# AIS-Bonn/stillleben

Measured on AMD Instinct MI355X. Metric: scenes/sec (settle + 640x480 6-ch GT render), 20-obj YCB-like, higher is better.
Workload: dtype f32; 1 GPU; C2: 20 of 21 procedural YCB-like objects (8k verts/16k tris, 1024^2 texture each) per scene; per step and GPU 32768 scenes are staged (random stack), settled (100 frames x 4 substeps), framed (camera, light, shadow matrix) and rendered at 640x480 (rgb, coord+depth, class, instance, normals; shadows on, SSAO on) -- all four stages inside the timed region; render_chunk=512, objects=20, settle_streams=1, render_streams=2, pair_contact_budget=0, parallelism=1 GPU

## Files before the change

### stillleben_amd/csrc/slhip_raster_walk.h

```cpp
#pragma once

#include <stdint.h>

#if defined(__HIPCC__)
#define SLHIP_RW_HD __host__ __device__ __forceinline__
#else
#define SLHIP_RW_HD inline
#endif

namespace slhip_raster {

constexpr long long kNarrowMax = 1ll << 29;

SLHIP_RW_HD bool narrow_ok(long long ex, long long ey)
{
    const long long m = ex > ey ? ex : ey;
    return 256 * m <= kNarrowMax && ex * ey <= kNarrowMax;
}

template <class I>
SLHIP_RW_HD I edge_value(const int* X, const int* Y, int flipped, int i, int cx, int cy)
{
    const int a = (i + 1) % 3, b = (i + 2) % 3;
    const I e = I(X[b] - X[a]) * I(cy - Y[a]) - I(Y[b] - Y[a]) * I(cx - X[a]);
    return flipped ? -e : e;
}

template <class I>
struct Walk {
    I e[3];
    I row[3];
    I sx[3];
    I sy[3];
    int bias[3];

    SLHIP_RW_HD void start(const int* X, const int* Y, int flipped, const int* bias_, int px, int py)
    {
        const int cx = 256 * px + 128, cy = 256 * py + 128;
#pragma unroll
        for (int i = 0; i < 3; ++i) {
            const int a = (i + 1) % 3, b = (i + 2) % 3;
            const I dx = I(-256) * I(Y[b] - Y[a]), dy = I(256) * I(X[b] - X[a]);
            sx[i] = flipped ? -dx : dx;
            sy[i] = flipped ? -dy : dy;
            bias[i] = bias_[i];
            row[i] = edge_value<I>(X, Y, flipped, i, cx, cy) + I(bias_[i]);
            e[i] = row[i];
        }
    }
    SLHIP_RW_HD void step_x()
    {
        e[0] += sx[0]; e[1] += sx[1]; e[2] += sx[2];
    }
    SLHIP_RW_HD void next_row()
    {
        row[0] += sy[0]; row[1] += sy[1]; row[2] += sy[2];
        e[0] = row[0]; e[1] = row[1]; e[2] = row[2];
    }
    SLHIP_RW_HD bool inside() const { return (e[0] | e[1] | e[2]) >= I(0); }
    SLHIP_RW_HD I numerator(int i) const { return e[i] - I(bias[i]); }
};

template <class I>
SLHIP_RW_HD bool cover(const int* X, const int* Y, int flipped, const int* bias, int px, int py, I* num)
{
    const int cx = 256 * px + 128, cy = 256 * py + 128;
    bool in = true;
#pragma unroll
    for (int i = 0; i < 3; ++i) {
        const I e = edge_value<I>(X, Y, flipped, i, cx, cy);
        in = in && (e + I(bias[i]) >= I(0));
        num[i] = e;
    }
    return in;
}

}
```

### stillleben_amd/csrc/slhip_render.hip

```cpp
#include <algorithm>
#include <cmath>
#include <cstring>
#include <vector>
#include <type_traits>
#include "slhip_common.h"
#include "slhip_cubemap.h"
#include "slhip_raster_walk.h"
#include "slhip_tile_queue.h"

#ifndef SLHIP_RENDER_WAVES
#define SLHIP_RENDER_WAVES 0
#endif
#ifndef SLHIP_SHADE_WAVES
#define SLHIP_SHADE_WAVES 0
#endif
#ifndef SLHIP_SSAO_WAVES
#define SLHIP_SSAO_WAVES 0
#endif
#if SLHIP_RENDER_WAVES > 0
#define SLHIP_LIGHT_KERNEL __attribute__((amdgpu_waves_per_eu(1, SLHIP_RENDER_WAVES)))
#else
#define SLHIP_LIGHT_KERNEL
#endif
#if SLHIP_RENDER_WAVES > 0
// ... 396 lines not shown

__device__ __forceinline__ int wrapi(int i, int n)
{
    if ((n & (n - 1)) == 0) return i & (n - 1);
    int m = i % n;
    return m < 0 ? m + n : m;
}

__device__ __forceinline__ int wrap_coord(int i, int n, unsigned mode)
{
    if (mode == 1u) return min(max(i, 0), n - 1);
    if (mode == 2u) {
        const int m = wrapi(i, 2 * n);
        return m < n ? m : 2 * n - 1 - m;
    }
    return wrapi(i, n);
}

__device__ __forceinline__ void texel_rgba(const uint8_t* __restrict__ pool_tex, unsigned lvl, int w, int x, int y, float* out)
{
    const uchar4 t = *reinterpret_cast<const uchar4*>(pool_tex + (lvl + 4u * ((unsigned)y * (unsigned)w + (unsigned)x)));
    out[0] = slhip::unorm8(t.x); out[1] = slhip::unorm8(t.y); out[2] = slhip::unorm8(t.z); out[3] = slhip::unorm8(t.w);
}

__device__ __forceinline__ void tex_level(const uint8_t* __restrict__ pool_tex, unsigned lvl, int w, int h, unsigned sampler,
                                          bool linear, float u, float v, float* out)
{
    const unsigned ws = SLHIP_SAMPLER_WRAP_S(sampler), wt = SLHIP_SAMPLER_WRAP_T(sampler);
    if (!linear) {
        texel_rgba(pool_tex, lvl, w, wrap_coord((int)floorf(u * (float)w), w, ws), wrap_coord((int)floorf(v * (float)h), h, wt), out);
        return;
    }
    const float x = fmaf(u, (float)w, -0.5f), y = fmaf(v, (float)h, -0.5f);
    const float fx = floorf(x), fy = floorf(y);
    const float ax = x - fx, ay = y - fy;
    const int x0 = wrap_coord((int)fx, w, ws), y0 = wrap_coord((int)fy, h, wt);
    const int x1 = wrap_coord((int)fx + 1, w, ws), y1 = wrap_coord((int)fy + 1, h, wt);
    float c00[4], c10[4], c01[4], c11[4];
    texel_rgba(pool_tex, lvl, w, x0, y0, c00); texel_rgba(pool_tex, lvl, w, x1, y0, c10);
    texel_rgba(pool_tex, lvl, w, x0, y1, c01); texel_rgba(pool_tex, lvl, w, x1, y1, c11);
#pragma unroll
    for (int c = 0; c < 4; ++c) {
        const float top = fmaf(ax, c10[c] - c00[c], c00[c]), bot = fmaf(ax, c11[c] - c01[c], c01[c]);
        out[c] = fmaf(ay, bot - top, top);
    }
}

__device__ __forceinline__ unsigned tex_level_off(unsigned tex, int w0, int h0, int l, int& w, int& h)
{
    unsigned off = tex;
    w = w0; h = h0;
    for (int k = 0; k < l; ++k) {
        off += 4u * (unsigned)w * (unsigned)h;
        w = max(1, w >> 1); h = max(1, h >> 1);
    }
    return off;
}

__device__ __forceinline__ float det_log2(float x)
{
    const unsigned bits = __float_as_uint(x);
    const int e = (int)(bits >> 23) - 127;
    const float t = __uint_as_float((bits & 0x7fffffu) | 0x3f800000u) - 1.0f;
    float q = 0.02049034833908081f;
    q = fmaf(q, t, -0.09606625884771347f);
    q = fmaf(q, t, 0.2155885398387909f);
    q = fmaf(q, t, -0.33924779295921326f);
    q = fmaf(q, t, 0.4777059257030487f);
    q = fmaf(q, t, -0.721162736415863f);
    q = fmaf(q, t, 1.4426932334899902f);
    return fmaf(q, t, (float)e);
}

__device__ __forceinline__ void tex_sample(const uint8_t* __restrict__ pool_tex, unsigned tex, int w, int h, unsigned sampler, float u,
                                           float v, float dudx, float dvdx, float dudy, float dvdy, float* out)
{
    const unsigned mip = SLHIP_SAMPLER_MIP(sampler);
    const float ax = dudx * (float)w, bx = dvdx * (float)h, ay = dudy * (float)w, by = dvdy * (float)h;
    const float rx = sqrtf(fmaf(bx, bx, ax * ax)), ry = sqrtf(fmaf(by, by, ay * ay));
    const float rho = fmaxf(rx, ry);
    const bool magnify = !(rho > 1.0f);
    if (magnify || mip == 0u) {
        tex_level(pool_tex, tex, w, h, sampler, (sampler & (magnify ? SLHIP_SAMPLER_MAG_LINEAR : SLHIP_SAMPLER_MIN_LINEAR)) != 0u, u, v, out);
        return;
    }
    const int top = 31 - __clz(max(max(w, h), 1));
    const float lambda = fminf(det_log2(rho), (float)top);
    const bool lin = (sampler & SLHIP_SAMPLER_MIN_LINEAR) != 0u;
    int lw, lh;
    if (mip == 1u) {
        const int l = min((int)ceilf(lambda + 0.5f) - 1, top);
        const unsigned p = tex_level_off(tex, w, h, max(l, 0), lw, lh);
        tex_level(pool_tex, p, lw, lh, sampler, lin, u, v, out);
        return;
    }
    const int l0 = min((int)floorf(lambda), top), l1 = min(l0 + 1, top);
    const float f = lambda - (float)l0;
    float a[4], b[4];
    const unsigned p0 = tex_level_off(tex, w, h, l0, lw, lh);
    tex_level(pool_tex, p0, lw, lh, sampler, lin, u, v, a);
    if (l1 == l0 || f == 0.0f) {
#pragma unroll
        for (int c = 0; c < 4; ++c) out[c] = a[c];
        return;
    }
    const unsigned p1 = p0 + 4u * (unsigned)lw * (unsigned)lh;
    lw = max(1, lw >> 1); lh = max(1, lh >> 1);
    tex_level(pool_tex, p1, lw, lh, sampler, lin, u, v, b);
#pragma unroll
    for (int c = 0; c < 4; ++c) out[c] = fmaf(f, b[c] - a[c], a[c]);
}

__device__ __forceinline__ void bary_at(const Setup& t, const float* b0, const float* b1, const float* b2, int px, int py, float* b)
{
    const int cx = 256 * px + 128, cy = 256 * py + 128;
    float l[3];
    const float fa = (float)t.area2;
#pragma unroll
    for (int i = 0; i < 3; ++i) {
        const int a = (i + 1) % 3, c = (i + 2) % 3;
        long long e = (long long)(t.X[c] - t.X[a]) * (long long)(cy - t.Y[a]) - (long long)(t.Y[c] - t.Y[a]) * (long long)(cx - t.X[a]);
        if (t.flipped) e = -e;
        l[i] = (float)e / fa;
    }
    const float pw0 = l[0] * t.invw[0], pw1 = l[1] * t.invw[1], pw2 = l[2] * t.invw[2];
    const float sw = (pw0 + pw1) + pw2;
    const float bs[3] = {pw0 * (1.0f / sw), pw1 * (1.0f / sw), pw2 * (1.0f / sw)};
#pragma unroll
    for (int k = 0; k < 3; ++k) b[k] = fmaf(bs[2], b2[k], fmaf(bs[1], b1[k], bs[0] * b0[k]));
}

__device__ __forceinline__ void tex_rect_bilinear(const uint8_t* __restrict__ tex, int w, int h, float xt, float yt, float* out)
{
    const float x = xt - 0.5f, y = yt - 0.5f;
    const float fx = floorf(x), fy = floorf(y);
    const float ax = x - fx, ay = y - fy;
    const int x0 = min(max((int)fx, 0), w - 1), x1 = min(max((int)fx + 1, 0), w - 1);
    const int y0 = (h - 1) - min(max((int)fy, 0), h - 1), y1 = (h - 1) - min(max((int)fy + 1, 0), h - 1);
    const uchar4 t00 = reinterpret_cast<const uchar4*>(tex)[(size_t)y0 * w + x0];
    const uchar4 t10 = reinterpret_cast<const uchar4*>(tex)[(size_t)y0 * w + x1];
    const uchar4 t01 = reinterpret_cast<const uchar4*>(tex)[(size_t)y1 * w + x0];
    const uchar4 t11 = reinterpret_cast<const uchar4*>(tex)[(size_t)y1 * w + x1];
    const unsigned char c00[4] = {t00.x, t00.y, t00.z, t00.w}, c10[4] = {t10.x, t10.y, t10.z, t10.w};
    const unsigned char c01[4] = {t01.x, t01.y, t01.z, t01.w}, c11[4] = {t11.x, t11.y, t11.z, t11.w};
#pragma unroll
    for (int c = 0; c < 4; ++c) {
        const float a = slhip::unorm8(c00[c]), b = slhip::unorm8(c10[c]);
        const float cc = slhip::unorm8(c01[c]), d = slhip::unorm8(c11[c]);
        const float top = fmaf(ax, b - a, a), bot = fmaf(ax, d - cc, cc);
        out[c] = fmaf(ay, bot - top, top);
    }
}

struct MainTarget {
    unsigned long long* vis;
    const float* peel;
    int W;
    unsigned prim;
    bool need_attr;
    const float* camz;
    const float* bary;
    const float* uv;
    const uint8_t* pool_tex;
    unsigned tex;
    int tex_w, tex_h;
    unsigned tex_sampler;
    float base_alpha, alpha_cutoff;

    __device__ __forceinline__ void emit(const Setup& t, int px, int py, const float* l) const
    {
        const float z = interp(l, t.z[0], t.z[1], t.z[2]);
        if (!(z >= 0.0f && z <= 1.0f)) return;
        const unsigned d24 = depth24(z);
        if (d24 >= 0xFFFFFFu) return;
        const unsigned long long key = ((unsigned long long)d24 << 32) | prim;
        unsigned long long* slot = vis + (size_t)py * W + px;
        if (need_attr && __builtin_nontemporal_load(slot) <= key) return;
        if (need_attr) {
            const float pw0 = l[0] * t.invw[0], pw1 = l[1] * t.invw[1], pw2 = l[2] * t.invw[2];
            const float sw = (pw0 + pw1) + pw2;
            const float bs[3] = {pw0 * (1.0f / sw), pw1 * (1.0f / sw), pw2 * (1.0f / sw)};
            float b[3];
#pragma unroll
            for (int k = 0; k < 3; ++k)
                b[k] = fmaf(bs[2], bary[6 + k], fmaf(bs[1], bary[3 + k], bs[0] * bary[k]));
            if (peel) {
                const float cz = interp(b, camz[0], camz[1], camz[2]);
                if (cz - 0.00001f <= peel[4 * ((size_t)py * W + px) + 3]) return;
            }
            if (pool_tex) {
                const float u = interp(b, uv[0], uv[2], uv[4]);
                const float v = interp(b, uv[1], uv[3], uv[5]);
                float bx[3], by[3];
                bary_at(t, bary, bary + 3, bary + 6, px + 1, py, bx);
                bary_at(t, bary, bary + 3, bary + 6, px, py + 1, by);
                float tc[4];
                tex_sample(pool_tex, tex, tex_w, tex_h, tex_sampler, u, v, interp(bx, uv[0], uv[2], uv[4]) - u, interp(bx, uv[1], uv[3], uv[5]) - v,
                           interp(by, uv[0], uv[2], uv[4]) - u, interp(by, uv[1], uv[3], uv[5]) - v, tc);
                if (base_alpha * tc[3] < alpha_cutoff) return;
            }
        }
        atomicMin(slot, key);
    }
};

#ifndef SLHIP_SHADOW_WINDOW
#define SLHIP_SHADOW_WINDOW 64
#endif
#ifndef SLHIP_SHADOW_WINDOW_PITCH
#define SLHIP_SHADOW_WINDOW_PITCH SLHIP_SHADOW_WINDOW
#endif
struct ShadowTarget {
    unsigned* sm;
    int W;
    unsigned* win;
    int wx0, wy0;
    unsigned wnx, wny;
    __device__ __forceinline__ void emit(const Setup& t, int px, int py, const float* l) const
    {
        const float z = interp(l, t.z[0], t.z[1], t.z[2]);
        if (!(z >= 0.0f && z <= 1.0f)) return;
        const unsigned bits = __float_as_uint(z);
#if SLHIP_SHADOW_WINDOW
        const unsigned ux = (unsigned)(px - wx0), uy = (unsigned)(py - wy0);
        if (ux < wnx && uy < wny) {
            atomicMin(win + uy * SLHIP_SHADOW_WINDOW_PITCH + ux, bits);
            return;
        }
#endif
        unsigned* slot = sm + (size_t)py * W + px;
        atomicMin(slot, bits);
    }
};

struct QueueShare {
    const slhip_tq::Entry* entries;
    slhip_tq::Walk walk;
    __device__ __forceinline__ QueueShare(const unsigned* __restrict__ queue, unsigned capacity)
    {
        const unsigned wave = (unsigned)__builtin_amdgcn_readfirstlane((int)((blockIdx.x * blockDim.x + threadIdx.x) >> 6));
        const unsigned n_waves = (gridDim.x * blockDim.x) >> 6;
        entries = reinterpret_cast<const slhip_tq::Entry*>(queue + slhip_tq::kHeaderWords);
        walk.first(slhip_tq::plan_of(queue[0], queue[1], queue[2], capacity), entries, n_waves, wave);
    }
};

struct TilePixels {
    unsigned ntx, tx, ty;
    int px0, py0;
    __device__ __forceinline__ TilePixels(const slhip_tq::Entry& en, unsigned k0, unsigned lane)
    {
        ntx = slhip_tq::ntx(en);
        ty = k0 / ntx; tx = k0 - ty * ntx;
        px0 = (int)((en.t0 & 0xFFFFu) << 3) + (int)(lane & 7);
        py0 = (int)((en.t0 >> 16) << 3) + (int)(lane >> 3);
    }
    __device__ __forceinline__ void next(int& px, int& py)
    {
        px = px0 + (int)(tx << 3); py = py0 + (int)(ty << 3);
        if (++tx == ntx) { tx = 0u; ++ty; }
    }
};

template <class I, class Target>
__device__ __forceinline__ void raster_bbox_as(const Setup& t, const Target& tgt)
{
    slhip_raster::Walk<I> w;
    w.start(t.X, t.Y, t.flipped, t.bias, t.xmin, t.ymin);
    const float fa = (float)(I)t.area2;
    const int bw = t.xmax - t.xmin + 1, n = bw * (t.ymax - t.ymin + 1);
    int px = t.xmin, py = t.ymin;
    for (int k = 0; k < n; ++k) {
        if (w.inside()) {
            float l[3];
            l[0] = (float)w.numerator(0) / fa;
            l[1] = (float)w.numerator(1) / fa;
            l[2] = (float)w.numerator(2) / fa;
            tgt.emit(t, px, py, l);
        }
        if (px == t.xmax) {
            px = t.xmin; ++py;
            w.next_row();
        } else {
            ++px;
            w.step_x();
        }
    }
}

template <class Target>
__device__ __forceinline__ void raster_bbox(const Setup& t, const Target& tgt, int wide)
{
    if (!wide && __all(t.narrow)) {
        raster_bbox_as<int>(t, tgt);
    } else {
        const int bw = t.xmax - t.xmin + 1, n = bw * (t.ymax - t.ymin + 1);
        int px = t.xmin, py = t.ymin;
        for (int k = 0; k < n; ++k) {
            float l[3];
            if (coverage_as<long long>(t, px, py, l)) tgt.emit(t, px, py, l);
            if (px == t.xmax) { px = t.xmin; ++py; } else ++px;
        }
    }
}

template <class Target>
__device__ __forceinline__ void raster_or_enqueue(const Setup& t, const Target& tgt, unsigned* queue,
                                                  unsigned capacity, unsigned draw, unsigned tri_sub,
                                                  unsigned scene_aux, int small_area, int wide = 0)
{
    const int bw = t.xmax - t.xmin + 1, bh = t.ymax - t.ymin + 1;
    bool in_place = bw * bh <= small_area;
    if (!in_place) {
        const unsigned tx0 = (unsigned)(t.xmin >> 3), ty0 = (unsigned)(t.ymin >> 3);
        const unsigned ntx = (unsigned)(t.xmax >> 3) - tx0 + 1u, nty = (unsigned)(t.ymax >> 3) - ty0 + 1u;
        const unsigned n = ntx * nty;
        const slhip_tq::Slot s =
            slhip_tq::slot_of(atomicAdd(reinterpret_cast<unsigned long long*>(queue), slhip_tq::reservation(n)), n, capacity);
        if (s.carried) atomicOr(queue + 2, 1u);
        if (s.fits) {
            uint4* e = reinterpret_cast<uint4*>(queue + slhip_tq::kHeaderWords) + slhip_tq::kUnitsPerEntry * (size_t)s.index;
            e[0] = make_uint4(draw, tri_sub, scene_aux, s.tile_base);
            e[1] = make_uint4(tx0 | (ty0 << 16), s.carried ? 0u : (ntx | (nty << 16)), 0u, 0u);
        }
        in_place = !s.fits || s.carried;
    }
    if (in_place) raster_bbox(t, tgt, wide);
}

template <bool kAttr>
__device__ __forceinline__ void raster_chunk(unsigned chunk, const slhip_mesh_pool& pool, const slhip_scene* __restrict__ scenes,
                                             const slhip_draw* __restrict__ draws,
                                             const slhip_chunk* __restrict__ chunks, int W, int H,
                                             const float* __restrict__ depth_peel,
                                             unsigned long long* __restrict__ vis, unsigned* queue,
                                             unsigned capacity, const float4* __restrict__ clipbuf,
                                             const uint4* __restrict__ screen, int small_area, int wide)
{
    const slhip_chunk ch = chunks[chunk];
    if (threadIdx.x >= ch.count) return;
    const slhip_scene* sc = scenes + ch.scene;
    const slhip_draw* dr = draws + ch.draw;
    const bool alpha_test = (dr->flags & SLHIP_DRAW_ALPHA_TEST) && (dr->flags & SLHIP_DRAW_HAS_BASE_TEX);
    if ((alpha_test || depth_peel != nullptr) != kAttr) return;
    const unsigned tri = ch.first_tri + threadIdx.x;
    const unsigned* ip = pool.d_idx + dr->idx_base + 3 * (size_t)tri;
    const unsigned vi[3] = {ip[0], ip[1], ip[2]};
    const size_t P = (size_t)W * H;
    MainTarget tgt;
    tgt.vis = vis + (size_t)ch.scene * P;
    tgt.W = W;
    tgt.prim = dr->prim_base + tri;
    tgt.need_attr = kAttr;
    tgt.peel = nullptr;
    tgt.pool_tex = nullptr;

    if constexpr (!kAttr) {
        tgt.camz = nullptr; tgt.uv = nullptr; tgt.bary = nullptr;
        const uint4 s0 = screen[dr->clip_base + vi[0]], s1 = screen[dr->clip_base + vi[1]], s2 = screen[dr->clip_base + vi[2]];
        if (screen_all_inside(s0, s1, s2)) {
            Setup t;
            if (setup_from_screen(s0, s1, s2, W, H, t)) raster_or_enqueue(t, tgt, queue, capacity, ch.draw, tri, ch.scene, small_area, wide);
            return;
        }
        ClipVert cv[3];
#pragma unroll
        for (int k = 0; k < 3; ++k) {
            const float4 c4 = clipbuf[dr->clip_base + vi[k]];
            cv[k].clip[0] = c4.x; cv[k].clip[1] = c4.y; cv[k].clip[2] = c4.z; cv[k].clip[3] = c4.w;
            cv[k].bary[0] = cv[k].bary[1] = cv[k].bary[2] = 0.0f;
        }
        ClipVert poly[4];
        const int n = clip_near(cv, poly);
#pragma unroll
        for (int sub = 0; sub < 2; ++sub) {
            if (sub >= n - 2) break;
            Setup t;
            if (!setup_tri(poly[0].clip, poly[sub + 1].clip, poly[sub + 2].clip, W, H, t)) continue;
            raster_or_enqueue(t, tgt, queue, capacity, ch.draw, tri | ((unsigned)sub << 31), ch.scene, small_area, wide);
        }
    } else {
        ClipVert cv[3];
        float camz[3] = {0.0f, 0.0f, 0.0f};
#pragma unroll
        for (int k = 0; k < 3; ++k) {
            const float4 c4 = clipbuf[dr->clip_base + vi[k]];
            cv[k].clip[0] = c4.x; cv[k].clip[1] = c4.y; cv[k].clip[2] = c4.z; cv[k].clip[3] = c4.w;
            if (depth_peel) {
                float unused[4];
                vertex_clip(pool, sc, dr, dr->vtx_base + vi[k], unused, camz[k]);
            }
            cv[k].bary[0] = k == 0 ? 1.0f : 0.0f;
            cv[k].bary[1] = k == 1 ? 1.0f : 0.0f;
            cv[k].bary[2] = k == 2 ? 1.0f : 0.0f;
        }
        ClipVert poly[4];
        const int n = clip_near(cv, poly);
        if (n == 0) return;
        tgt.peel = depth_peel ? depth_peel + 4 * (size_t)ch.scene * P : nullptr;
        float uvs[6] = {0, 0, 0, 0, 0, 0};
        if (alpha_test) {
#pragma unroll
            for (int k = 0; k < 3; ++k) {
                const float2 uv = reinterpret_cast<const float2*>(pool.d_uv)[dr->vtx_base + vi[k]];
                uvs[2 * k] = uv.x; uvs[2 * k + 1] = uv.y;
            }
            tgt.pool_tex = pool.d_tex; tgt.tex = dr->tex_offset;
            tgt.tex_w = (int)dr->tex_w; tgt.tex_h = (int)dr->tex_h;
            tgt.tex_sampler = dr->tex_sampler[0];
        }
        tgt.camz = camz;
        tgt.uv = uvs;
        tgt.base_alpha = dr->base_color[3];
        tgt.alpha_cutoff = dr->alpha_cutoff;
#pragma unroll
        for (int sub = 0; sub < 2; ++sub) {
            if (sub >= n - 2) break;
            Setup t;
            if (!setup_tri(poly[0].clip, poly[sub + 1].clip, poly[sub + 2].clip, W, H, t)) continue;
            float bary[9];
#pragma unroll
            for (int k = 0; k < 3; ++k) {
                bary[k] = poly[0].bary[k];
                bary[3 + k] = poly[sub + 1].bary[k];
                bary[6 + k] = poly[sub + 2].bary[k];
            }
            tgt.bary = bary;
            for (int py = t.ymin; py <= t.ymax; ++py)
                for (int px = t.xmin; px <= t.xmax; ++px) {
                    float l[3];
                    if (coverage(t, px, py, l)) tgt.emit(t, px, py, l);
                }
        }
    }
}

template <bool kAttr>
__global__ __launch_bounds__(256) SLHIP_LIGHT_KERNEL void k_raster(slhip_mesh_pool pool, const slhip_scene* __restrict__ scenes,
                                                const slhip_draw* __restrict__ draws,
                                                const slhip_chunk* __restrict__ chunks, unsigned n_chunks, int W, int H,
                                                const float* __restrict__ depth_peel,
                                                unsigned long long* __restrict__ vis, unsigned* queue,
                                                unsigned capacity, const float4* __restrict__ clipbuf,
                                                const uint4* __restrict__ screen, int small_area, int wide)
{
    for (unsigned c = blockIdx.x; c < n_chunks; c += gridDim.x)
        raster_chunk<kAttr>(c, pool, scenes, draws, chunks, W, H, depth_peel, vis, queue, capacity, clipbuf, screen, small_area, wide);
}

__global__ __launch_bounds__(256) SLHIP_LIGHT_KERNEL void k_large(slhip_mesh_pool pool, const slhip_scene* __restrict__ scenes,
                                               const slhip_draw* __restrict__ draws, int W, int H,
                                               unsigned long long* __restrict__ vis,
                                               const unsigned* __restrict__ queue, unsigned capacity,
                                               const float4* __restrict__ clipbuf, const uint4* __restrict__ screen)
{
    const QueueShare q(queue, capacity);
    const unsigned lane = threadIdx.x & 63;
    for (unsigned e = q.walk.e0; e < q.walk.e1; ++e) {
        const slhip_tq::Entry en = q.entries[e];
        if (q.walk.done(en)) break;
        unsigned k0, k1;
        if (!q.walk.tiles(en, k0, k1)) continue;
        Setup t;
        const slhip_draw* dr = draws + en.draw;
        const unsigned tri = en.tri_sub & 0x7FFFFFFFu;
        const int sub = (int)(en.tri_sub >> 31);
        const unsigned* ip = pool.d_idx + dr->idx_base + 3 * (size_t)tri;
        ClipVert cv[3];
        const uint4 s0 = screen[dr->clip_base + ip[0]], s1 = screen[dr->clip_base + ip[1]], s2 = screen[dr->clip_base + ip[2]];
        const bool cached = screen_all_inside(s0, s1, s2);
        if (cached && (sub != 0 || !setup_from_screen(s0, s1, s2, W, H, t))) continue;
        if (!cached) {
#pragma unroll
            for (int k = 0; k < 3; ++k) {
                const float4 c4 = clipbuf[dr->clip_base + ip[k]];
                cv[k].clip[0] = c4.x; cv[k].clip[1] = c4.y; cv[k].clip[2] = c4.z; cv[k].clip[3] = c4.w;
                cv[k].bary[0] = cv[k].bary[1] = cv[k].bary[2] = 0.0f;
            }
            ClipVert poly[4];
            const int n = clip_near(cv, poly);
            if (sub > n - 3) continue;
            const ClipVert& pb = sub == 0 ? poly[1] : poly[2];
            const ClipVert& pc = sub == 0 ? poly[2] : poly[3];
            if (!setup_tri(poly[0].clip, pb.clip, pc.clip, W, H, t)) continue;
        }
        MainTarget tgt;
        tgt.vis = vis + (size_t)en.scene_aux * W * H;
        tgt.peel = nullptr;
        tgt.W = W;
        tgt.prim = dr->prim_base + tri;
        tgt.need_attr = false;
        tgt.pool_tex = nullptr;
        TilePixels tp(en, k0, lane);
        for (unsigned k = k0; k < k1; ++k) {
            int px, py;
            tp.next(px, py);
            if (px < t.xmin || px > t.xmax || py < t.ymin || py > t.ymax) continue;
            float l[3];
            if (!coverage(t, px, py, l)) continue;
            tgt.emit(t, px, py, l);
        }
    }
}

__device__ __forceinline__ void shadow_clip(const slhip_mesh_pool& pool, const float* T, unsigned v, float* clip)
{
    const float4 p = reinterpret_cast<const float4*>(pool.d_pos)[v];
    const float pos[4] = {p.x, p.y, p.z, 1.0f};
#pragma unroll
    for (int r = 0; r < 4; ++r) {
        float a = fmaf(T[4 * r + 0], pos[0], 0.0f);
        a = fmaf(T[4 * r + 1], pos[1], a);
        a = fmaf(T[4 * r + 2], pos[2], a);
        a = fmaf(T[4 * r + 3], pos[3], a);
        clip[r] = a;
    }
}

template <bool kMax>
__device__ __forceinline__ int wave_minmax(int v)
{
    constexpr int ident = kMax ? (int)0x80000000 : 0x7fffffff;
#define SLHIP_DPP_STEP(ctrl, rows)                                                       \
    {                                                                                    \
        const int o = __builtin_amdgcn_update_dpp(ident, v, ctrl, rows, 0xf, false);     \
        v = kMax ? max(v, o) : min(v, o);                                                \
    }
    SLHIP_DPP_STEP(0x111, 0xf) SLHIP_DPP_STEP(0x112, 0xf) SLHIP_DPP_STEP(0x114, 0xf) SLHIP_DPP_STEP(0x118, 0xf)
    SLHIP_DPP_STEP(0x142, 0xa) SLHIP_DPP_STEP(0x143, 0xc)
#undef SLHIP_DPP_STEP
    return __builtin_amdgcn_readlane(v, 63);
}

constexpr int kShadowTile = 64;
constexpr int kShadowMaxWords = 32;
__host__ __device__ inline int shadow_tiles_x(int S) { return (S + kShadowTile - 1) / kShadowTile; }
__host__ __device__ inline int shadow_tile_words(int S) { return (shadow_tiles_x(S) * shadow_tiles_x(S) + 31) / 32; }

__global__ __launch_bounds__(256) SLHIP_SHADOW_RASTER_KERNEL void k_shadow_raster(slhip_mesh_pool pool, const slhip_scene* __restrict__ scenes,
                                                       const slhip_draw* __restrict__ draws,
                                                       const slhip_chunk* __restrict__ chunks, int S,
                                                       unsigned* __restrict__ shadow, unsigned* queue,
                                                       unsigned capacity, const float4* __restrict__ clipbuf,
                                                       unsigned n_clip_verts, unsigned* __restrict__ tile_bits, int nl,
                                                       int small_area, int wide)
{
    __shared__ unsigned bm[SLHIP_NUM_LIGHTS][kShadowMaxWords];
    const slhip_chunk ch = chunks[blockIdx.x];
    if (ch.count == 0) return;
    const slhip_scene* sc = scenes + ch.scene;
    const slhip_draw* dr = draws + ch.draw;
    if (!(dr->flags & SLHIP_DRAW_CASTS_SHADOW)) return;
    const int tx_n = shadow_tiles_x(S), words = shadow_tile_words(S);
    for (int k = (int)threadIdx.x; k < SLHIP_NUM_LIGHTS * kShadowMaxWords; k += 256) bm[k / kShadowMaxWords][k % kShadowMaxWords] = 0u;
#if SLHIP_SHADOW_WINDOW
    __shared__ int4 wbox[SLHIP_NUM_LIGHTS][4];
#endif
    __syncthreads();
    const bool have_tri = threadIdx.x < ch.count;
    const unsigned tri = ch.first_tri + (have_tri ? threadIdx.x : 0u);
    const unsigned* ip = pool.d_idx + dr->idx_base + 3 * (size_t)tri;
    const unsigned i0 = ip[0], i1 = ip[1], i2 = ip[2];
#if SLHIP_SHADOW_WINDOW
    constexpr int kWin = SLHIP_SHADOW_WINDOW;
    constexpr int kPitch = SLHIP_SHADOW_WINDOW_PITCH;
    __shared__ unsigned win[kWin * kPitch];
#endif
    for (int light = 0; light < nl; ++light) {
        if (!light_active(sc, light)) continue;
        const float4* plane = clipbuf + (size_t)(1 + light) * n_clip_verts + dr->clip_base;
        Setup t;
        const uint4* sp = reinterpret_cast<const uint4*>(plane);
        bool draw = have_tri && setup_from_screen(sp[i0], sp[i1], sp[i2], S, S, t);
        if (draw && t.flipped) draw = false;
#if SLHIP_SHADOW_WINDOW
        {
            const bool walks = draw && (t.xmax - t.xmin + 1) * (t.ymax - t.ymin + 1) <= small_area;
            const int bx0 = wave_minmax<false>(walks ? t.xmin : 0x7fffffff), by0 = wave_minmax<false>(walks ? t.ymin : 0x7fffffff);
            const int bx1 = wave_minmax<true>(walks ? t.xmax : -1), by1 = wave_minmax<true>(walks ? t.ymax : -1);
            if ((threadIdx.x & 63u) == 0u) wbox[light][threadIdx.x >> 6] = make_int4(bx0, by0, bx1, by1);
        }
        __syncthreads();
        const int4 b0 = wbox[light][0], b1 = wbox[light][1], b2 = wbox[light][2], b3 = wbox[light][3];
        const int wx0 = min(min(b0.x, b1.x), min(b2.x, b3.x)), wy0 = min(min(b0.y, b1.y), min(b2.y, b3.y));
        const bool have_win = wx0 != 0x7fffffff;
        unsigned wnx = 0u, wny = 0u, wsh = 0u;
        if (have_win) {
            wnx = (unsigned)max(min(max(max(b0.z, b1.z), max(b2.z, b3.z)) - wx0 + 1, kWin), 1);
            wny = (unsigned)max(min(max(max(b0.w, b1.w), max(b2.w, b3.w)) - wy0 + 1, kWin), 1);
            wsh = 32u - (unsigned)__clz((int)wnx - 1);
            const unsigned n = wny << wsh, cmask = (1u << wsh) - 1u;
            for (unsigned k = threadIdx.x; k < n; k += 256) win[(k >> wsh) * kPitch + (k & cmask)] = 0x3F800000u;
            __syncthreads();
        }
#endif
        if (draw) {
            if (words <= kShadowMaxWords) {
                const int tx0 = t.xmin / kShadowTile, tx1 = t.xmax / kShadowTile, ty0 = t.ymin / kShadowTile, ty1 = t.ymax / kShadowTile;
                for (int ty = ty0; ty <= ty1; ++ty)
                    for (int tx = tx0; tx <= tx1; ++tx) {
// ... 1254 lines not shown
        return -1;
    }
    counts[0] = counts[1] = 0;
    if (width % 32 != 0 || height % 16 != 0 || n_scenes == 0) return 0;
    const uint64_t nt = (uint64_t)n_scenes * ssao_tiles_per_scene(width, height);
    std::vector<unsigned char> h(nt);
    const char* base = reinterpret_cast<const char*>(scratch->d_ao) + ssao_tiles_offset(n_scenes, width, height) + nt * 8;
    SLHIP_CHECK(hipMemcpyAsync(h.data(), base, nt, hipMemcpyDeviceToHost, stream));
    SLHIP_CHECK(hipStreamSynchronize(stream));
    counts[0] = nt;
    for (unsigned char b : h) counts[1] += b & 1;
    return 0;
}

extern "C" int slhip_render_ssao_levels(const slhip_render_scratch* scratch, uint32_t n_scenes, uint32_t width, uint32_t height,
                                        uint64_t counts[8], void* stream_)
{
    hipStream_t stream = (hipStream_t)stream_;
    if (!scratch || !scratch->d_ao || !counts) {
        slhip::set_error("slhip_render_ssao_levels: null argument");
        return -1;
    }
    for (int i = 0; i < 8; ++i) counts[i] = 0;
    if (width % 32 != 0 || height % 16 != 0 || n_scenes == 0) return 0;
    const uint64_t nt = (uint64_t)n_scenes * ssao_tiles_per_scene(width, height);
    std::vector<unsigned char> h(nt);
    unsigned stats[2] = {0, 0};
    const char* ao = reinterpret_cast<const char*>(scratch->d_ao);
    SLHIP_CHECK(hipMemcpyAsync(h.data(), ao + ssao_tiles_offset(n_scenes, width, height) + nt * 8, nt, hipMemcpyDeviceToHost, stream));
    SLHIP_CHECK(hipMemcpyAsync(stats, ao + ssao_stats_offset(n_scenes, width, height), sizeof(stats), hipMemcpyDeviceToHost, stream));
    SLHIP_CHECK(hipStreamSynchronize(stream));
    for (unsigned char b : h) counts[std::min<int>(b >> 1, kSsaoLevels - 1)] += 1;
    counts[6] = stats[0];
    counts[7] = stats[1];
    return 0;
}

constexpr int kSsaoBandRows = 16;
static unsigned ssao_band_rows_knob()
{
    const char* e = getenv("SLHIP_SSAO_BAND_ROWS");
    const int v = e ? atoi(e) : kSsaoBandRows;
    return (unsigned)std::min(std::max(16, v / 16 * 16), 1 << 16);
}

extern "C" int slhip_render(const slhip_mesh_pool* pool, const slhip_scene* d_scenes, const slhip_draw* d_draws,
                            const slhip_chunk* d_chunks, uint32_t n_scenes, uint32_t n_draws, uint32_t n_chunks,
                            uint32_t width,
                            uint32_t height, uint32_t flags, const float* d_depth_peel,
                            const slhip_render_out* out, const slhip_render_scratch* scratch, void* stream_)
{
    hipStream_t stream = (hipStream_t)stream_;
    if (!pool || !d_scenes || !d_draws || !out || !scratch) {
        slhip::set_error("slhip_render: null argument");
        return -1;
    }
    if (n_scenes == 0 || width == 0 || height == 0) return 0;
    if (!scratch->d_vis || !scratch->d_queue) {
        slhip::set_error("slhip_render: d_vis and d_queue scratch are required");
        return -1;
    }
    const bool want_rgb = out->d_rgb != nullptr;
    const bool ssao = (flags & SLHIP_RENDER_SSAO) && want_rgb;
    const bool shadows = (flags & SLHIP_RENDER_SHADOWS) && want_rgb && scratch->d_shadow != nullptr;
    if (shadows && (!scratch->d_shadow_tiles || (scratch->shadow_res & 3u))) {
        slhip::set_error("slhip_render: shadows need the d_shadow_tiles scratch and a shadow_res that is a multiple of 4");
        return -1;
    }
    if (ssao && (!out->d_cam_coord || !out->d_normals || !scratch->d_ao)) {
        slhip::set_error("slhip_render: SSAO needs the cam_coord and normals outputs and d_ao scratch");
        return -1;
    }
    if (want_rgb && (!scratch->d_hdr || !scratch->d_lum)) {
        slhip::set_error("slhip_render: rgb output needs d_hdr and d_lum scratch");
        return -1;
    }
    const int W = (int)width, H = (int)height;
    const size_t P = (size_t)W * H;
    const unsigned blocks_per_scene = (unsigned)((P + 255) / 256);
    const unsigned pix_blocks = blocks_per_scene * 8u * ((n_scenes + 7u) / 8u);
    const int S = (int)scratch->shadow_res;
    const int raster_small = getenv("SLHIP_RASTER_SMALL") ? atoi(getenv("SLHIP_RASTER_SMALL")) : kSmallArea;
    const int shadow_small = getenv("SLHIP_SHADOW_SMALL") ? atoi(getenv("SLHIP_SHADOW_SMALL")) : kSmallArea;
    const int raster_wide = getenv("SLHIP_RASTER_WIDE") ? atoi(getenv("SLHIP_RASTER_WIDE")) : 0;
    const int NL = scratch->shadow_lights == 0u ? SLHIP_NUM_LIGHTS : (int)min(scratch->shadow_lights, (uint32_t)SLHIP_NUM_LIGHTS);
    if (n_chunks > 0 && (!scratch->d_clip || scratch->n_clip_verts == 0)) {
        slhip::set_error("slhip_render: d_clip scratch (n_clip_verts x 16 B x planes) is required");
        return -1;
    }
    if (n_chunks > 0 && !scratch->d_vattr) {
        slhip::set_error("slhip_render: d_vattr scratch (n_clip_verts x 80 B) is required");
        return -1;
    }
    const float4* clipbuf = reinterpret_cast<const float4*>(scratch->d_clip);
    float4* vattr = reinterpret_cast<float4*>(scratch->d_vattr);
    const uint4* screen = reinterpret_cast<const uint4*>(vattr) + 4 * (size_t)scratch->n_clip_verts;

    if (ssao) {
        int dev = 0;
        SLHIP_CHECK(hipGetDevice(&dev));
        if (dev < 16 && !g_ssao_tables_uploaded[dev]) {
            SLHIP_CHECK(hipMemcpyToSymbolAsync(HIP_SYMBOL(c_ssao_noise), k_ssao_noise_host, sizeof(float) * 48, 0,
                                               hipMemcpyHostToDevice, stream));
            SLHIP_CHECK(hipMemcpyToSymbolAsync(HIP_SYMBOL(c_ssao_kernel), k_ssao_kernel_host, sizeof(float) * 192, 0,
                                               hipMemcpyHostToDevice, stream));
            const SsaoLevelTables& lt = ssao_level_tables();
            if (lt.count.n[0] != 0) {
                slhip::set_error("slhip_render: the first SSAO level threshold does not cover the longest kernel sample");
                return -1;
            }
            SLHIP_CHECK(hipMemcpyToSymbolAsync(HIP_SYMBOL(c_ssao_level_kernel), lt.kern, sizeof(lt.kern), 0, hipMemcpyHostToDevice, stream));
            g_ssao_tables_uploaded[dev] = true;
        }
    }

    if (g_timing) {
        constexpr size_t kMaxTimedCalls = 4096;
        if (g_timed.size() >= kMaxTimedCalls) {
            const size_t drop = g_timed.size() / 2;
            for (size_t k = 0; k < drop; ++k)
                for (int i = 0; i <= kNumPhases; ++i)
                    if (g_timed[k].recorded[i]) (void)hipEventDestroy(g_timed[k].ev[i]);
            g_timed.erase(g_timed.begin(), g_timed.begin() + (long)drop);
        }
        g_timed.emplace_back();
        g_cur = &g_timed.back();
        for (int i = 0; i <= kNumPhases; ++i) g_cur->recorded[i] = false;
    }
    if (n_chunks > 0) {
        k_vertex_xform<<<dim3(n_draws, 32), 256, 0, stream>>>(*pool, d_scenes, d_draws, reinterpret_cast<float4*>(scratch->d_clip),
                                                                      scratch->n_clip_verts, vattr, W, H, shadows ? 1 : 0, S);
        SLHIP_LAUNCH_CHECK();
    }
    const unsigned n_tile_words = shadows ? n_scenes * SLHIP_NUM_LIGHTS * (unsigned)shadow_tile_words(S) : 0u;
    if (shadows && (flags & SLHIP_RENDER_SHADOW_RESET)) {
        k_clear_shadow<<<4096, 256, 0, stream>>>(reinterpret_cast<unsigned*>(scratch->d_shadow),
                                                 (size_t)n_scenes * NL * S * S / 4);
        SLHIP_CHECK(hipMemsetAsync(scratch->d_shadow_tiles, 0, (size_t)n_tile_words * 4, stream));
    }
    if (shadows && n_chunks > 0) {
        mark(0, stream);
        SLHIP_CHECK(hipMemsetAsync(scratch->d_queue, 0, 16, stream));
        k_shadow_raster<<<n_chunks, 256, 0, stream>>>(
            *pool, d_scenes, d_draws, d_chunks, S, reinterpret_cast<unsigned*>(scratch->d_shadow),
            scratch->d_queue, scratch->queue_capacity, clipbuf, scratch->n_clip_verts, scratch->d_shadow_tiles, NL, shadow_small, raster_wide);
        mark(1, stream);
        k_shadow_large<<<2048, 256, 0, stream>>>(*pool, d_scenes, d_draws, S,
                                                 reinterpret_cast<unsigned*>(scratch->d_shadow), scratch->d_queue,
                                                 scratch->queue_capacity, clipbuf, scratch->n_clip_verts, NL, raster_wide);
        SLHIP_LAUNCH_CHECK();
    }

    mark(2, stream);
    SLHIP_CHECK(hipMemsetAsync(scratch->d_vis, 0xFF, (size_t)n_scenes * P * 8, stream));
    SLHIP_CHECK(hipMemsetAsync(scratch->d_queue, 0, 16, stream));
    if (n_chunks > 0) {
        if (!d_depth_peel)
            k_raster<false><<<n_chunks, 256, 0, stream>>>(*pool, d_scenes, d_draws, d_chunks, n_chunks, W, H, d_depth_peel,
                                                          reinterpret_cast<unsigned long long*>(scratch->d_vis),
                                                          scratch->d_queue, scratch->queue_capacity, clipbuf, screen, raster_small, raster_wide);
        k_raster<true><<<d_depth_peel ? n_chunks : min(n_chunks, 4096u), 256, 0, stream>>>(
            *pool, d_scenes, d_draws, d_chunks, n_chunks, W, H, d_depth_peel, reinterpret_cast<unsigned long long*>(scratch->d_vis),
            scratch->d_queue, scratch->queue_capacity, clipbuf, screen, raster_small, raster_wide);
        mark(3, stream);
        k_large<<<2048, 256, 0, stream>>>(*pool, d_scenes, d_draws, W, H,
                                          reinterpret_cast<unsigned long long*>(scratch->d_vis), scratch->d_queue,
                                          scratch->queue_capacity, clipbuf, screen);
        SLHIP_LAUNCH_CHECK();
    }

    ShadeParams prm;
    prm.W = W; prm.H = H; prm.n_scenes = n_scenes; prm.flags = flags; prm.S = S; prm.shadow_lights = NL;
    prm.inline_tonemap = 0;
    prm.want_lum = want_rgb ? 1 : 0;
    static const int shade_tiled = getenv("SLHIP_SHADE_TILED") ? atoi(getenv("SLHIP_SHADE_TILED")) : 1;
    prm.tiled = (shade_tiled && W % 32 == 0 && H % 8 == 0) ? 1 : 0;
    float* hdr0 = want_rgb ? scratch->d_hdr : nullptr;
    float* hdr1 = want_rgb ? scratch->d_hdr + 4 * (size_t)n_scenes * P : nullptr;
    mark(4, stream);
    static const int ssao_tiled_on = getenv("SLHIP_SSAO_TILED") ? atoi(getenv("SLHIP_SSAO_TILED")) : 1;
    const bool ssao_tiled = ssao && want_rgb && ssao_tiled_on && prm.tiled && H % 16 == 0 && W % 32 == 0 && (W / 8 + 1) * (H / 8 + 1) * 4 <= 60000;
    float2* ssao_tiles = ssao_tiled ? reinterpret_cast<float2*>(reinterpret_cast<char*>(scratch->d_ao) + ssao_tiles_offset(n_scenes, W, H)) : nullptr;
    unsigned char* ssao_skip = ssao_tiled ? reinterpret_cast<unsigned char*>(ssao_tiles + (size_t)n_scenes * ssao_tiles_per_scene(W, H)) : nullptr;
    const int shade_reference = getenv("SLHIP_SHADE_REFERENCE") ? atoi(getenv("SLHIP_SHADE_REFERENCE")) : 0;
    auto launch_shade = [&](auto kernel) {
        kernel<<<pix_blocks, 256, 0, stream>>>(*pool, d_scenes, d_draws, prm,
                                               reinterpret_cast<const unsigned long long*>(scratch->d_vis), *out, hdr0,
                                               shadows ? scratch->d_shadow : nullptr, scratch->d_lum, clipbuf,
                                               ssao ? scratch->d_ao + (size_t)n_scenes * P : nullptr, vattr, ssao_tiles,
                                               shadows && !getenv("SLHIP_NO_PCF_TILES") ? scratch->d_shadow_tiles : nullptr);
    };
    if (shade_reference) launch_shade(k_shade<true>);
    else launch_shade(k_shade<false>);
    SLHIP_LAUNCH_CHECK();
    if (shadows && n_chunks > 0) {
        k_shadow_restore<<<n_tile_words, 256, 0, stream>>>(reinterpret_cast<unsigned*>(scratch->d_shadow), scratch->d_shadow_tiles,
                                                          S, n_tile_words, NL);
        SLHIP_LAUNCH_CHECK();
    }

    if (want_rgb) {
        k_lum_reduce<<<n_scenes, 256, 0, stream>>>(d_scenes, (unsigned)((P + 255) / 256), P, scratch->d_lum);
        if (ssao) {
            mark(5, stream);
            const float* zpl = scratch->d_ao + (size_t)n_scenes * P;
            const float* d_kernel_table = nullptr;
            SLHIP_CHECK(hipGetSymbolAddress((void**)&d_kernel_table, HIP_SYMBOL(c_ssao_kernel)));
            if (ssao_tiled) {
                const unsigned band_rows = ssao_band_rows_knob();
                const int ssao_dbg = getenv("SLHIP_SSAO_DEBUG") ? atoi(getenv("SLHIP_SSAO_DEBUG")) : 0;
                const unsigned bands = ((unsigned)H + band_rows - 1u) / band_rows;
                unsigned* drain_stats = reinterpret_cast<unsigned*>(reinterpret_cast<char*>(scratch->d_ao) + ssao_stats_offset(n_scenes, W, H));
                const float* d_level_table = nullptr;
                SLHIP_CHECK(hipGetSymbolAddress((void**)&d_level_table, HIP_SYMBOL(c_ssao_level_kernel)));
                k_ssao_mask<<<n_scenes, 256, (size_t)(W / 8 + 1) * (H / 8 + 1) * 4, stream>>>(d_scenes, W, H, ssao_tiles, ssao_skip, ssao_dbg, drain_stats);
                k_ssao_tiled<<<8u * ((n_scenes + 7u) / 8u) * bands * 4u, 256, 0, stream>>>(d_scenes, n_scenes, W, H, out->d_cam_coord, out->d_normals,
                                                                                   zpl, scratch->d_ao, d_level_table, ssao_level_tables().count, ssao_skip,
                                                                                   band_rows, ssao_dbg == 3 ? drain_stats : nullptr);
            } else
                k_ssao<<<pix_blocks, 256, 0, stream>>>(d_scenes, n_scenes, W, H, out->d_cam_coord, out->d_normals, zpl, scratch->d_ao,
                                                       d_kernel_table);
            mark(6, stream);
            k_ssao_apply<<<pix_blocks, 256, 0, stream>>>(d_scenes, n_scenes, W, H, hdr0, scratch->d_ao, zpl,
                                                         (flags & SLHIP_RENDER_KEEP_HDR) ? hdr1 : nullptr, scratch->d_lum, out->d_rgb, ssao_skip);
            mark(7, stream);
        } else {
            mark(7, stream);
            k_tonemap<<<pix_blocks, 256, 0, stream>>>(d_scenes, n_scenes, W, H, hdr0, scratch->d_lum, out->d_rgb);
        }
        SLHIP_LAUNCH_CHECK();
    }
    mark(kNumPhases, stream);
    return 0;
}

#include "slhip_render_stats.inc"
#include "slhip_render_masks.inc"
```

### stillleben_amd/csrc/slhip_tile_queue.h

```cpp
#pragma once

#include <stdint.h>

#if defined(__HIPCC__)
#define SLHIP_TQ_HD __host__ __device__ __forceinline__
#else
#define SLHIP_TQ_HD inline
#endif

namespace slhip_tq {

constexpr unsigned kHeaderWords = 4;
constexpr unsigned kUnitsPerEntry = 2;

struct Entry {
    unsigned draw;
    unsigned tri_sub;
    unsigned scene_aux;
    unsigned tile_base;
    unsigned t0;
    unsigned nt;
    unsigned spare[2];
};
static_assert(sizeof(Entry) == 16 * kUnitsPerEntry, "an entry is two 16-byte units");

SLHIP_TQ_HD unsigned entry_capacity(unsigned capacity_units) { return capacity_units / kUnitsPerEntry; }
SLHIP_TQ_HD unsigned ntx(const Entry& e) { return e.nt & 0xFFFFu; }
SLHIP_TQ_HD unsigned nty(const Entry& e) { return e.nt >> 16; }
SLHIP_TQ_HD unsigned n_tiles(const Entry& e) { return ntx(e) * nty(e); }

SLHIP_TQ_HD unsigned long long reservation(unsigned n) { return 1ull | ((unsigned long long)n << 32); }

struct Slot {
    unsigned index;
    unsigned tile_base;
    bool fits;
    bool carried;
};
SLHIP_TQ_HD Slot slot_of(unsigned long long before, unsigned n, unsigned capacity_units)
{
    Slot s;
    s.index = (unsigned)before;
    s.tile_base = (unsigned)(before >> 32);
    s.fits = s.index < entry_capacity(capacity_units);
    s.carried = (unsigned long long)s.tile_base + n > 0xFFFFFFFFull;
    return s;
}

struct Plan {
    unsigned count;
    unsigned total;
    bool by_entries;
};
SLHIP_TQ_HD Plan plan_of(unsigned entries, unsigned tiles, unsigned carried, unsigned capacity_units)
{
    Plan p;
    const unsigned cap = entry_capacity(capacity_units);
    p.count = entries < cap ? entries : cap;
    p.by_entries = carried != 0u;
    p.total = p.by_entries ? p.count : tiles;
    if (p.count == 0u) p.total = 0u;
    return p;
}

SLHIP_TQ_HD void range_of(unsigned total, unsigned n_ranges, unsigned r, unsigned& t0, unsigned& t1)
{
    const unsigned long long per = ((unsigned long long)total + n_ranges - 1) / n_ranges;
    const unsigned long long a = per * r, b = a + per;
    t0 = (unsigned)(a < total ? a : total);
    t1 = (unsigned)(b < total ? b : total);
}

SLHIP_TQ_HD unsigned find_entry(const Entry* entries, unsigned count, unsigned t)
{
    unsigned lo = 0, hi = count;
    while (hi - lo > 1u) {
        const unsigned mid = lo + (hi - lo) / 2;
        if (entries[mid].tile_base <= t) lo = mid; else hi = mid;
    }
    return lo;
}

struct Walk {
    unsigned t0, t1;
    unsigned e0, e1;
    bool by_entries;

    SLHIP_TQ_HD void first(const Plan& p, const Entry* entries, unsigned n_ranges, unsigned r)
    {
        by_entries = p.by_entries;
        unsigned a, b;
        range_of(p.total, n_ranges, r, a, b);
        if (by_entries) {
            e0 = a; e1 = b; t0 = 0u; t1 = 0xFFFFFFFFu;
        } else {
            t0 = a; t1 = b; e1 = p.count;
            e0 = a < b ? find_entry(entries, p.count, a) : p.count;
        }
    }
    SLHIP_TQ_HD bool done(const Entry& e) const { return !by_entries && e.tile_base >= t1; }
    SLHIP_TQ_HD bool tiles(const Entry& e, unsigned& k0, unsigned& k1) const
    {
        const unsigned n = n_tiles(e);
        if (by_entries) { k0 = 0u; k1 = n; return n != 0u; }
        const unsigned base = e.tile_base, end = base + n;
        const unsigned lo = t0 > base ? t0 : base, hi = t1 < end ? t1 : end;
        if (lo >= hi) return false;
        k0 = lo - base; k1 = hi - base;
        return true;
    }
};

}
```

Measured before the change: 10920 scenes/s.

## Fuse vis-buffer clear with rasterizing tiny scenes' few plain triangles

Replaces the vis-buffer memset with a fill kernel. For scenes whose plain (non-alpha-tested) draws total at most four triangles, the kernel rasterizes those triangles directly while clearing, and the chunk rasterizer then skips those draws. It also adds a queue flag so the attribute raster pass exits early when no chunk needs it. For the 20-object 16k-triangle workload, few scenes qualify. The fill kernel adds per-scene setup, a loop over the draws, and writes in place of a plain memset.

```diff
diff --git a/stillleben_amd/csrc/slhip_raster_walk.h b/stillleben_amd/csrc/slhip_raster_walk.h
--- a/stillleben_amd/csrc/slhip_raster_walk.h
+++ b/stillleben_amd/csrc/slhip_raster_walk.h
@@ -57,6 +57,11 @@
         row[0] += sy[0]; row[1] += sy[1]; row[2] += sy[2];
         e[0] = row[0]; e[1] = row[1]; e[2] = row[2];
     }
+    SLHIP_RW_HD void rows_down(int n)
+    {
+        row[0] += I(n) * sy[0]; row[1] += I(n) * sy[1]; row[2] += I(n) * sy[2];
+        e[0] = row[0]; e[1] = row[1]; e[2] = row[2];
+    }
     SLHIP_RW_HD bool inside() const { return (e[0] | e[1] | e[2]) >= I(0); }
     SLHIP_RW_HD I numerator(int i) const { return e[i] - I(bias[i]); }
 };
diff --git a/stillleben_amd/csrc/slhip_render.hip b/stillleben_amd/csrc/slhip_render.hip
--- a/stillleben_amd/csrc/slhip_render.hip
+++ b/stillleben_amd/csrc/slhip_render.hip
@@ -572,6 +572,16 @@
     }
 }
 
+__device__ __forceinline__ bool fragment_key(const Setup& t, const float* l, unsigned prim, unsigned long long& key)
+{
+    const float z = interp(l, t.z[0], t.z[1], t.z[2]);
+    if (!(z >= 0.0f && z <= 1.0f)) return false;
+    const unsigned d24 = depth24(z);
+    if (d24 >= 0xFFFFFFu) return false;
+    key = ((unsigned long long)d24 << 32) | prim;
+    return true;
+}
+
 struct MainTarget {
     unsigned long long* vis;
     const float* peel;
@@ -589,11 +599,8 @@
 
     __device__ __forceinline__ void emit(const Setup& t, int px, int py, const float* l) const
     {
-        const float z = interp(l, t.z[0], t.z[1], t.z[2]);
-        if (!(z >= 0.0f && z <= 1.0f)) return;
-        const unsigned d24 = depth24(z);
-        if (d24 >= 0xFFFFFFu) return;
-        const unsigned long long key = ((unsigned long long)d24 << 32) | prim;
+        unsigned long long key;
+        if (!fragment_key(t, l, prim, key)) return;
         unsigned long long* slot = vis + (size_t)py * W + px;
         if (need_attr && __builtin_nontemporal_load(slot) <= key) return;
         if (need_attr) {
@@ -748,6 +755,26 @@
     if (in_place) raster_bbox(t, tgt, wide);
 }
 
+constexpr unsigned kFillMaxTris = 4;
+__device__ __forceinline__ bool fill_plain(unsigned flags, unsigned n_tris)
+{
+    return !((flags & SLHIP_DRAW_ALPHA_TEST) && (flags & SLHIP_DRAW_HAS_BASE_TEX)) && n_tris <= 2u;
+}
+__device__ __forceinline__ bool fill_draw(const slhip_scene* sc, const slhip_draw* __restrict__ draws, unsigned d, unsigned flags,
+                                          unsigned n_tris, bool depth_peel)
+{
+    if (depth_peel || !fill_plain(flags, n_tris)) return false;
+    const unsigned begin = sc->draw_begin, end = sc->draw_end;
+    if (d < begin || d >= end) return false;
+    unsigned n = 0;
+#pragma unroll 2
+    for (unsigned j = begin; j < end; ++j) {
+        const unsigned f = draws[j].flags, t = draws[j].n_tris;
+        n += fill_plain(f, t) ? t : 0u;
+    }
+    return n <= kFillMaxTris;
+}
+
 template <bool kAttr>
 __device__ __forceinline__ void raster_chunk(unsigned chunk, const slhip_mesh_pool& pool, const slhip_scene* __restrict__ scenes,
                                              const slhip_draw* __restrict__ draws,
@@ -755,14 +782,21 @@
                                              const float* __restrict__ depth_peel,
                                              unsigned long long* __restrict__ vis, unsigned* queue,
                                              unsigned capacity, const float4* __restrict__ clipbuf,
-                                             const uint4* __restrict__ screen, int small_area, int wide)
+                                             const uint4* __restrict__ screen, int small_area, int wide, int fill)
 {
     const slhip_chunk ch = chunks[chunk];
     if (threadIdx.x >= ch.count) return;
     const slhip_scene* sc = scenes + ch.scene;
     const slhip_draw* dr = draws + ch.draw;
-    const bool alpha_test = (dr->flags & SLHIP_DRAW_ALPHA_TEST) && (dr->flags & SLHIP_DRAW_HAS_BASE_TEX);
-    if ((alpha_test || depth_peel != nullptr) != kAttr) return;
+    const unsigned draw_flags = dr->flags;
+    const bool alpha_test = (draw_flags & SLHIP_DRAW_ALPHA_TEST) && (draw_flags & SLHIP_DRAW_HAS_BASE_TEX);
+    if ((alpha_test || depth_peel != nullptr) != kAttr) {
+        if constexpr (!kAttr)
+            if ((fill & 2) && threadIdx.x == 0) atomicOr(queue + slhip_tq::kFlagWord, slhip_tq::kFlagDiscardChunks);
+        return;
+    }
+    if constexpr (!kAttr)
+        if ((fill & 1) && ch.count <= 2u && fill_draw(sc, draws, ch.draw, draw_flags, dr->n_tris, false)) return;
     const unsigned tri = ch.first_tri + threadIdx.x;
     const unsigned* ip = pool.d_idx + dr->idx_base + 3 * (size_t)tri;
     const unsigned vi[3] = {ip[0], ip[1], ip[2]};
@@ -862,10 +896,131 @@
                                                 const float* __restrict__ depth_peel,
                                                 unsigned long long* __restrict__ vis, unsigned* queue,
                                                 unsigned capacity, const float4* __restrict__ clipbuf,
-                                                const uint4* __restrict__ screen, int small_area, int wide)
-{
+                                                const uint4* __restrict__ screen, int small_area, int wide, int fill)
+{
+    if constexpr (kAttr)
+        if ((fill & 2) && depth_peel == nullptr && queue[slhip_tq::kFlagWord] == 0u) return;
     for (unsigned c = blockIdx.x; c < n_chunks; c += gridDim.x)
-        raster_chunk<kAttr>(c, pool, scenes, draws, chunks, W, H, depth_peel, vis, queue, capacity, clipbuf, screen, small_area, wide);
+        raster_chunk<kAttr>(c, pool, scenes, draws, chunks, W, H, depth_peel, vis, queue, capacity, clipbuf, screen, small_area, wide, fill);
+}
+
+__device__ __forceinline__ bool scene_block(unsigned blocks_per_scene, unsigned n_scenes, unsigned& scene, unsigned& blk);
+constexpr int kFillRows = 8;
+struct FillList {
+    Setup t[2 * kFillMaxTris];
+    unsigned prim[2 * kFillMaxTris];
+    unsigned tri[kFillMaxTris][2];
+    unsigned n_tri, n_sub;
+};
+__device__ __forceinline__ int uniform_i(int v) { return __builtin_amdgcn_readfirstlane(v); }
+__device__ __forceinline__ float uniform_f(float v) { return __int_as_float(__builtin_amdgcn_readfirstlane(__float_as_int(v))); }
+__device__ __forceinline__ void uniform_setup(const Setup& s, Setup& t)
+{
+#pragma unroll
+    for (int i = 0; i < 3; ++i) {
+        t.X[i] = uniform_i(s.X[i]); t.Y[i] = uniform_i(s.Y[i]); t.bias[i] = uniform_i(s.bias[i]);
+        t.z[i] = uniform_f(s.z[i]); t.invw[i] = uniform_f(s.invw[i]);
+    }
+    t.area2 = (long long)(((unsigned long long)(unsigned)uniform_i((int)(s.area2 >> 32)) << 32) | (unsigned)uniform_i((int)s.area2));
+    t.flipped = uniform_i(s.flipped); t.narrow = uniform_i(s.narrow);
+    t.xmin = uniform_i(s.xmin); t.xmax = uniform_i(s.xmax); t.ymin = uniform_i(s.ymin); t.ymax = uniform_i(s.ymax);
+}
+
+__global__ __launch_bounds__(256) SLHIP_LIGHT_KERNEL void k_vis_fill(slhip_mesh_pool pool, const slhip_scene* __restrict__ scenes,
+                                                  const slhip_draw* __restrict__ draws, unsigned n_scenes, int W, int H,
+                                                  unsigned rows_per_block, int geometry, unsigned long long* __restrict__ vis,
+                                                  const float4* __restrict__ clipbuf, const uint4* __restrict__ screen)
+{
+    __shared__ FillList s;
+    const unsigned col_strips = ((unsigned)W + 63u) >> 6, row_strips = ((unsigned)H + rows_per_block - 1u) / rows_per_block;
+    unsigned scene, blk;
+    if (!scene_block(col_strips * row_strips, n_scenes, scene, blk)) return;
+    if (threadIdx.x == 0) { s.n_tri = 0u; s.n_sub = 0u; }
+    __syncthreads();
+    if (geometry) {
+        const slhip_scene* sc = scenes + scene;
+        for (unsigned d = sc->draw_begin + threadIdx.x; d < sc->draw_end; d += blockDim.x) {
+            const unsigned n = draws[d].n_tris;
+            if (fill_draw(sc, draws, d, draws[d].flags, n, false)) {
+                const unsigned base = atomicAdd(&s.n_tri, n);
+                for (unsigned k = 0; k < n; ++k) { s.tri[base + k][0] = d; s.tri[base + k][1] = k; }
+            }
+        }
+        __syncthreads();
+        if (threadIdx.x < s.n_tri) {
+            const slhip_draw* dr = draws + s.tri[threadIdx.x][0];
+            const unsigned tri = s.tri[threadIdx.x][1];
+            const unsigned* ip = pool.d_idx + dr->idx_base + 3 * (size_t)tri;
+            const uint4 s0 = screen[dr->clip_base + ip[0]], s1 = screen[dr->clip_base + ip[1]], s2 = screen[dr->clip_base + ip[2]];
+            Setup t;
+            if (screen_all_inside(s0, s1, s2)) {
+                if (setup_from_screen(s0, s1, s2, W, H, t)) {
+                    const unsigned slot = atomicAdd(&s.n_sub, 1u);
+                    s.t[slot] = t; s.prim[slot] = dr->prim_base + tri;
+                }
+            } else {
+                ClipVert cv[3];
+#pragma unroll
+                for (int k = 0; k < 3; ++k) {
+                    const float4 c4 = clipbuf[dr->clip_base + ip[k]];
+                    cv[k].clip[0] = c4.x; cv[k].clip[1] = c4.y; cv[k].clip[2] = c4.z; cv[k].clip[3] = c4.w;
+                    cv[k].bary[0] = cv[k].bary[1] = cv[k].bary[2] = 0.0f;
+                }
+                ClipVert poly[4];
+                const int n = clip_near(cv, poly);
+#pragma unroll
+                for (int sub = 0; sub < 2; ++sub) {
+                    if (sub >= n - 2) break;
+                    if (!setup_tri(poly[0].clip, poly[sub + 1].clip, poly[sub + 2].clip, W, H, t)) continue;
+                    const unsigned slot = atomicAdd(&s.n_sub, 1u);
+                    s.t[slot] = t; s.prim[slot] = dr->prim_base + tri;
+                }
+            }
+        }
+        __syncthreads();
+    }
+    const int n_sub = uniform_i((int)s.n_sub);
+    const unsigned cs = blk % col_strips, rs = blk / col_strips;
+    const int x0 = (int)(cs << 6), px = x0 + (int)(threadIdx.x & 63u);
+    const int wave = uniform_i((int)(threadIdx.x >> 6));
+    const int row_begin = (int)(rs * rows_per_block), row_end = min(H, row_begin + (int)rows_per_block);
+    unsigned long long* out = vis + (size_t)scene * W * H;
+    for (int r0 = row_begin; r0 < row_end; r0 += 4 * kFillRows) {
+        const int py0 = r0 + wave, py_last = py0 + 4 * (kFillRows - 1);
+        unsigned long long key[kFillRows];
+#pragma unroll
+        for (int k = 0; k < kFillRows; ++k) key[k] = kVisEmpty;
+        for (int i = 0; i < n_sub; ++i) {
+            if (x0 + 63 < uniform_i(s.t[i].xmin) || x0 > uniform_i(s.t[i].xmax) || py_last < uniform_i(s.t[i].ymin) ||
+                py0 > uniform_i(s.t[i].ymax))
+                continue;
+            Setup t;
+            uniform_setup(s.t[i], t);
+            const unsigned prim = (unsigned)uniform_i((int)s.prim[i]);
+            slhip_raster::Walk<long long> w;
+            w.start(t.X, t.Y, t.flipped, t.bias, px, py0);
+            const float fa = (float)t.area2;
+            const bool in_columns = px >= t.xmin && px <= t.xmax;
+#pragma unroll
+            for (int k = 0; k < kFillRows; ++k) {
+                const int py = py0 + 4 * k;
+                if (in_columns && py >= t.ymin && py <= t.ymax && w.inside()) {
+                    float l[3];
+                    l[0] = (float)w.numerator(0) / fa;
+                    l[1] = (float)w.numerator(1) / fa;
+                    l[2] = (float)w.numerator(2) / fa;
+                    unsigned long long kk;
+                    if (fragment_key(t, l, prim, kk)) key[k] = min(key[k], kk);
+                }
+                w.rows_down(4);
+            }
+        }
+#pragma unroll
+        for (int k = 0; k < kFillRows; ++k) {
+            const int py = py0 + 4 * k;
+            if (px < W && py < row_end) out[(size_t)py * W + px] = key[k];
+        }
+    }
 }
 
 __global__ __launch_bounds__(256) SLHIP_LIGHT_KERNEL void k_large(slhip_mesh_pool pool, const slhip_scene* __restrict__ scenes,
@@ -2426,16 +2581,25 @@
     }
 
     mark(2, stream);
-    SLHIP_CHECK(hipMemsetAsync(scratch->d_vis, 0xFF, (size_t)n_scenes * P * 8, stream));
+    const int vis_fill = getenv("SLHIP_VIS_FILL") ? atoi(getenv("SLHIP_VIS_FILL")) : (getenv("SLHIP_RASTER_SMALL") ? 2 : 3);
+    if (vis_fill & 1) {
+        const unsigned rows_per_block = 96u;
+        const unsigned strips = (((unsigned)W + 63u) >> 6) * (((unsigned)H + rows_per_block - 1u) / rows_per_block);
+        k_vis_fill<<<strips * 8u * ((n_scenes + 7u) / 8u), 256, 0, stream>>>(
+            *pool, d_scenes, d_draws, n_scenes, W, H, rows_per_block, n_chunks > 0 && !d_depth_peel ? 1 : 0,
+            reinterpret_cast<unsigned long long*>(scratch->d_vis), clipbuf, screen);
+        SLHIP_LAUNCH_CHECK();
+    } else
+        SLHIP_CHECK(hipMemsetAsync(scratch->d_vis, 0xFF, (size_t)n_scenes * P * 8, stream));
     SLHIP_CHECK(hipMemsetAsync(scratch->d_queue, 0, 16, stream));
     if (n_chunks > 0) {
         if (!d_depth_peel)
             k_raster<false><<<n_chunks, 256, 0, stream>>>(*pool, d_scenes, d_draws, d_chunks, n_chunks, W, H, d_depth_peel,
                                                           reinterpret_cast<unsigned long long*>(scratch->d_vis),
-                                                          scratch->d_queue, scratch->queue_capacity, clipbuf, screen, raster_small, raster_wide);
+                                                          scratch->d_queue, scratch->queue_capacity, clipbuf, screen, raster_small, raster_wide, vis_fill);
         k_raster<true><<<d_depth_peel ? n_chunks : min(n_chunks, 4096u), 256, 0, stream>>>(
             *pool, d_scenes, d_draws, d_chunks, n_chunks, W, H, d_depth_peel, reinterpret_cast<unsigned long long*>(scratch->d_vis),
-            scratch->d_queue, scratch->queue_capacity, clipbuf, screen, raster_small, raster_wide);
+            scratch->d_queue, scratch->queue_capacity, clipbuf, screen, raster_small, raster_wide, vis_fill);
         mark(3, stream);
         k_large<<<2048, 256, 0, stream>>>(*pool, d_scenes, d_draws, W, H,
                                           reinterpret_cast<unsigned long long*>(scratch->d_vis), scratch->d_queue,
diff --git a/stillleben_amd/csrc/slhip_tile_queue.h b/stillleben_amd/csrc/slhip_tile_queue.h
--- a/stillleben_amd/csrc/slhip_tile_queue.h
+++ b/stillleben_amd/csrc/slhip_tile_queue.h
@@ -12,6 +12,8 @@
 
 constexpr unsigned kHeaderWords = 4;
 constexpr unsigned kUnitsPerEntry = 2;
+constexpr unsigned kFlagWord = 3;
+constexpr unsigned kFlagDiscardChunks = 1u;
 
 struct Entry {
     unsigned draw;
```

Result: faster. 11070 scenes/s (median of 6 runs) (+1.4%).
